# kdavila/lecturemath

Measured on AMD Instinct MI355X. Metric: frames/sec end-to-end binarize+CC+group @1080p, higher is better.
Workload: dtype u8

## Files before the change

### include/lecturemath_amd.h

```cpp
#ifndef LECTUREMATH_AMD_H
#define LECTUREMATH_AMD_H

#include <stdint.h>

#ifdef __cplusplus
extern "C" {
#endif

#define LM_OK 0
#define LM_ERR_ARG 1
#define LM_ERR_HIP 2
#define LM_ERR_CAPACITY 3
#define LM_ERR_STATE 4

typedef struct LmCtx LmCtx;
typedef struct LmStream LmStream;

int lm_abi_version(void);
const char* lm_last_error(void);
int lm_is_device_build(void);


int CC_AgeBoundaries(int* labels, float* ages, int width, int height, int count_labels,
                     int* out_mins_y, int* out_maxs_y, int* out_mins_x, int* out_maxs_x,
// ... 35 lines not shown
int lm_stream_push_records(LmStream* s, const uint8_t* d_binary, int n_frames, int32_t* d_labels, void* stream);
int lm_stream_match(LmStream* s, int n_frames, void* stream);
int lm_stream_push_labelled(LmStream* s, int n_frames, void* stream);

int lm_stream_run_logits(LmStream* s, const float* d_logits, int n_frames, int batch, uint8_t* d_binary, int32_t* d_labels, int thr,
                         int do_match, int schedule, void* stream_wide, void* stream_match);

int lm_stream_pack_size(LmStream* s, int first_frame, int n_frames, int64_t* h_bytes, void* stream);
int lm_stream_pack(LmStream* s, int first_frame, int n_frames, void* d_buf, int64_t bytes, void* stream);
int lm_stream_append_packed(LmStream* s, const void* d_buf, int64_t bytes, void* stream);

int lm_stream_assign_bytes(LmStream* s, int64_t* bytes, void* stream);
int lm_stream_export_assign(LmStream* s, void* d_out, int64_t bytes, void* stream);
int lm_stream_import_assign(LmStream* s, const void* d_in, int64_t bytes, void* stream);

int lm_stream_match_stats(LmStream* s, int64_t* out5, void* stream);

int lm_stream_counters(LmStream* s, int64_t* h_out7, void* stream);

int lm_stream_import(LmStream* s, const int32_t* h_rec, const int64_t* h_frame_off, const int64_t* h_crop_off,
                     const uint32_t* h_crop, int n_frames, int64_t n_cc, int64_t n_crop_words, int n_unique,
                     int64_t tempo_count, const int32_t* h_active, const int32_t* h_active_cc, const int32_t* h_active_last,
                     int n_active, int n_matched, void* stream);

int lm_stream_read(LmStream* s, int32_t* h_rec, int64_t* h_frame_off, int64_t* h_crop_off, uint32_t* h_crop,
                   int32_t* h_active, void* stream);

typedef struct LmGroups LmGroups;

LmGroups* lm_group_run(LmStream* s, int max_gap, int min_times, int t_window, double min_recall, double img_threshold,
                       int reconstruct_tables, void* stream);
// ... 63 lines not shown
```

### lecturemath_amd/csrc/lm_api.hip

```cpp
#include "lm_common.h"
#include "lm_stream.h"

#include <stdarg.h>
#include <stdlib.h>
#include <stdio.h>
#include <string.h>

#include "../../include/lecturemath_amd.h"

#include "lm_cc_kernels.hip"
#include "lm_match_kernels.hip"
#include "lm_match_batch.hip"
#include "lm_group.hip"
#include "lm_fcn.hip"
#include "lm_fcn2.hip"

static thread_local char g_err[512] = "";

void lm_set_error(const char* fmt, ...)
{
    va_list ap;
    va_start(ap, fmt);
    vsnprintf(g_err, sizeof(g_err), fmt, ap);
    va_end(ap);
// ... 479 lines not shown
    if (!ok) lm_set_error("CC_AgeBoundaries: device copy/launch failed");
    (void)hipFree(d_out);
    return 0;
}

extern "C" void lm_stream_destroy(LmStream* s)
{
    if (!s) return;
    void* ptrs[] = {s->cc, s->assign, s->frame_cc_off, s->crop, s->chash, s->active_cc, s->active_box, s->active_last, s->active, s->counters, s->best,
                    s->batch_cc_base, s->batch_word_base};
    for (void* p : ptrs)
        if (p) (void)hipFree(p);
    if (s->mb) {
        LmMatchBatch* m = s->mb;
        void* mp[] = {m->nt_cnt, m->nt_src, m->tlast, m->tcur[0], m->tcur[1], m->ftile_all, m->nt_foff, m->nt_list, m->cls, m->troot, m->rootpos, m->ftile, m->s_prefix, m->tcount[0], m->tcount[1], m->toff[0], m->toff[1], m->pairs[0], m->pairs[1], m->pair_u[0],
                      m->pair_u[1], m->sidx, m->s_list, m->s_box, m->newpos, m->n_src, m->ttab, m->tkey, m->twin, m->big[0], m->big[1], m->n_big};
        for (void* p : mp)
            if (p) (void)hipFree(p);
        delete m;
    }
    for (int i = 0; i < s->n_run_events; i++) (void)hipEventDestroy(s->run_events[i]);
    free(s->run_events);
    if (s->rd_scratch) (void)hipFree(s->rd_scratch);
    if (s->garena) (void)hipFree(s->garena);
    if (s->gpin) (void)hipHostFree(s->gpin);
    delete s;
}

extern "C" int lm_stream_set_min_pixels(LmStream* s, int min_pixels)
{
    if (!s || min_pixels < 0) { lm_set_error("lm_stream_set_min_pixels: bad arguments"); return LM_ERR_ARG; }
    s->min_pixels = min_pixels;
    return LM_OK;
}

extern "C" int lm_stream_reset(LmStream* s, void* stream)
{
    if (!s) { lm_set_error("lm_stream_reset: null stream"); return LM_ERR_ARG; }
    LM_HIP(hipMemsetAsync(s->counters, 0, sizeof(LmCounters), (hipStream_t)stream));
    LM_HIP(hipMemsetAsync(s->best, 0xff, (size_t)s->ctx->g.cap * sizeof(unsigned long long), (hipStream_t)stream));
    LM_HIP(hipMemsetAsync(s->frame_cc_off, 0, sizeof(long long), (hipStream_t)stream));
    LM_HIP(hipMemsetAsync(s->chash, 0, (size_t)s->cap_cc * sizeof(uint32_t), (hipStream_t)stream));
    if (s->mb) LM_HIP(hipMemsetAsync(s->mb->ttab, 0xff, (size_t)LM_MB_TTAB * sizeof(unsigned long long), (hipStream_t)stream));
    s->frames_pushed = 0;
    s->frames_matched = 0;
    s->tempo_B = 0;
    return LM_OK;
}

extern "C" LmStream* lm_stream_create(LmCtx* ctx, int max_frames, int64_t max_ccs, int64_t max_crop_words, int max_uniques,
                                      double min_recall, double min_precision, int max_gap, int min_pixels)
{
    if (!ctx || max_frames <= 0 || max_ccs <= 0 || max_crop_words <= 0 || max_uniques <= 0) {
        lm_set_error("lm_stream_create: bad arguments");
        return nullptr;
    }
    LmStream* s = new LmStream();
    memset(s, 0, sizeof(*s));
// ... 47 lines not shown
            rc |= lm_alloc(&m->pairs[k], (size_t)m->cap_pairs);
            rc |= lm_alloc(&m->pair_u[k], (size_t)m->cap_pairs);
        }
        rc |= lm_alloc(&m->sidx, (size_t)max_ccs);
        rc |= lm_alloc(&m->s_list, (size_t)max_ccs);
        rc |= lm_alloc(&m->s_box, (size_t)max_ccs);
        rc |= lm_alloc(&m->newpos, (size_t)max_ccs);
        rc |= lm_alloc(&m->n_src, (size_t)1);
        rc |= lm_alloc(&m->ttab, (size_t)LM_MB_TTAB);
        rc |= lm_alloc(&m->tkey, (size_t)max_ccs);
        rc |= lm_alloc(&m->twin, (size_t)max_ccs);
        m->cap_big = 1u << 16;
        rc |= lm_alloc(&m->big[0], (size_t)m->cap_big);
        rc |= lm_alloc(&m->big[1], (size_t)m->cap_big);
        rc |= lm_alloc(&m->n_big, (size_t)2);
#if !LM_HIP_EMULATED
        if (rc == LM_OK &&
            hipFuncSetAttribute((const void*)lm_k_mb_resolve, hipFuncAttributeMaxDynamicSharedMemorySize, (int)LM_MB_RESOLVE_SMEM) != hipSuccess)
            rc = LM_ERR_HIP;
#endif
        const char* e = getenv("LM_MATCH_PER_FRAME");
        s->match_per_frame = (e && atoi(e) == 1) ? 1 : 0;
    }
    if (rc == LM_OK && hipMemset(s->mb->twin, 0, (size_t)max_ccs) != hipSuccess) rc = LM_ERR_HIP;
    if (rc == LM_OK) rc = lm_stream_reset(s, nullptr);
    if (rc == LM_OK && hipStreamSynchronize(nullptr) != hipSuccess) rc = LM_ERR_HIP;
    if (rc != LM_OK) {
        lm_stream_destroy(s);
        return nullptr;
    }
// ... 28 lines not shown
    const dim3 gj(LM_HIP_EMULATED ? 2 : 128, LM_HIP_EMULATED ? 2 : LM_MB_JY), gt(LM_HIP_EMULATED ? 2 : 1024), ge(LM_HIP_EMULATED ? 2 : 2048), gb(LM_HIP_EMULATED ? 2 : 1024);
    for (int done = 0; done < n;) {
        const int B = (n - done < LM_MB_MAX_FRAMES) ? n - done : LM_MB_MAX_FRAMES;
        const int f = f0 + done;
        s->last_match_frames = B;
        const int twins = (s->min_recall <= 1.0 && s->min_precision <= 1.0) ? 1 : 0;
        if (twins) {
            const dim3 gc(LM_HIP_EMULATED ? 2 : 256);
            hipLaunchKernelGGL(lm_k_mb_twin_insert, gc, dim3(256), 0, st, s->cc, s->chash, s->frame_cc_off, f, B, s->counters, mb);
            hipLaunchKernelGGL(lm_k_mb_twin_probe, gc, dim3(256), 0, st, s->cc, s->frame_cc_off, f, B, s->counters, mb, s->max_gap);
            hipLaunchKernelGGL(lm_k_mb_twin_cmp, ge, dim3(256), 0, st, s->cc, s->crop, s->frame_cc_off, f, B, s->counters, mb);
            hipLaunchKernelGGL(lm_k_mb_twin_final, gc, dim3(256), 0, st, s->cc, s->frame_cc_off, f, B, s->counters, mb);
        }
        hipLaunchKernelGGL(lm_k_mb_nt, dim3(B + 1), dim3(1024), 0, st, s->frame_cc_off, f, B, s->active, s->active_cc, s->active_box, s->active_last,
                           s->counters, mb, s->max_gap, twins);
        hipLaunchKernelGGL((lm_k_mb_join<0, 0>), gj, dim3(256), 0, st, s->cc, s->frame_cc_off, f, B, s->active_box, s->active_cc, s->counters, mb);
        hipLaunchKernelGGL((lm_k_mb_join<0, 1>), gj, dim3(256), 0, st, s->cc, s->frame_cc_off, f, B, s->active_box, s->active_cc, s->counters, mb);
        hipLaunchKernelGGL((lm_k_mb_eval<0>), ge, dim3(256), 0, st, s->cc, s->crop, s->frame_cc_off, f, B, s->active_last, s->counters, mb,
                           s->min_recall, s->min_precision, s->max_gap);
        hipLaunchKernelGGL((lm_k_mb_eval_big<0>), gb, dim3(256), 0, st, s->cc, s->crop, s->active_last, s->counters, mb, s->min_recall, s->min_precision,
                           s->max_gap);
        hipLaunchKernelGGL(lm_k_mb_sources, dim3(1), dim3(1024), 0, st, s->cc, s->frame_cc_off, f, B, s->counters, mb);
        hipLaunchKernelGGL((lm_k_mb_join<1, 0>), gj, dim3(256), 0, st, s->cc, s->frame_cc_off, f, B, s->active_box, s->active_cc, s->counters, mb);
        hipLaunchKernelGGL((lm_k_mb_join<1, 1>), gj, dim3(256), 0, st, s->cc, s->frame_cc_off, f, B, s->active_box, s->active_cc, s->counters, mb);
        hipLaunchKernelGGL((lm_k_mb_eval<1>), ge, dim3(256), 0, st, s->cc, s->crop, s->frame_cc_off, f, B, s->active_last, s->counters, mb,
                           s->min_recall, s->min_precision, s->max_gap);
        hipLaunchKernelGGL((lm_k_mb_eval_big<1>), gb, dim3(256), 0, st, s->cc, s->crop, s->active_last, s->counters, mb, s->min_recall, s->min_precision,
                           s->max_gap);
        if (ev_pre && done + B >= n) (void)hipEventRecord(ev_pre, st);
        hipLaunchKernelGGL(lm_k_mb_resolve, dim3(1), dim3(LM_MB_RT), LM_MB_RESOLVE_SMEM, st, s->cc, s->frame_cc_off, f, B, s->active, s->active_cc,
                           s->active_box, s->active_last, s->counters, s->assign, mb, s->max_gap, s->cap_uniq);
        if (defer_tempo && done + B >= n) { s->tempo_f0 = f; s->tempo_B = B; }
        else
            hipLaunchKernelGGL(lm_k_mb_tempo, gt, dim3(256), 0, st, s->cc, s->frame_cc_off, f, B, s->active_box, s->active_cc, s->active_last,
                               s->counters, mb, s->max_gap, s->active, s->assign);
        done += B;
    }
}

// ... 142 lines not shown
    return LM_OK;
}

extern "C" int lm_stream_match(LmStream* s, int n_frames, void* stream)
{
    if (!s || n_frames < 0 || s->frames_matched + n_frames > s->frames_pushed) {
        lm_set_error("lm_stream_match: %d frames requested, %d pushed, %d matched", n_frames, s ? s->frames_pushed : 0, s ? s->frames_matched : 0);
        return LM_ERR_ARG;
    }
    lm_launch_match_frames(s, s->frames_matched, n_frames, (hipStream_t)stream);
    s->frames_matched += n_frames;
    LM_HIP(hipGetLastError());
    return LM_OK;
}

extern "C" int lm_stream_match_stats(LmStream* s, int64_t* out5, void* stream)
{
    if (!s || !out5 || !s->mb) { lm_set_error("lm_stream_match_stats: bad arguments"); return LM_ERR_ARG; }
    hipStream_t st = (hipStream_t)stream;
    const LmMatchBatch* m = s->mb;
    const int B = s->last_match_frames;
    int32_t nsrc = 0, nt = 0;
    uint32_t ta = 0, tb = 0;
    if (B > 0) {
        LM_HIP(hipMemcpyAsync(&nsrc, m->n_src, 4, hipMemcpyDeviceToHost, st));
        LM_HIP(hipMemcpyAsync(&nt, m->ftile + B, 4, hipMemcpyDeviceToHost, st));
        LM_HIP(hipStreamSynchronize(st));
        if (nt > 0) {
            LM_HIP(hipMemcpyAsync(&ta, m->toff[0] + nt, 4, hipMemcpyDeviceToHost, st));
            LM_HIP(hipMemcpyAsync(&tb, m->toff[1] + nt, 4, hipMemcpyDeviceToHost, st));
            LM_HIP(hipStreamSynchronize(st));
        }
    }
    out5[0] = nsrc; out5[1] = nt; out5[2] = ta; out5[3] = tb; out5[4] = B;
    return LM_OK;
}

__global__ void __launch_bounds__(1024) lm_k_compact_active(int32_t* __restrict__ active, int32_t* __restrict__ active_cc,
                                                            unsigned long long* __restrict__ active_box, int32_t* __restrict__ active_last,
                                                            LmCounters* __restrict__ cnt, int max_gap)
{
    if (cnt->error) return;
    const int f = cnt->n_matched;
    const int nA = cnt->n_active;
    if (f <= 1) return;
    unsigned kept = 0;
    for (int base = 0; base < nA; base += 1024) {
        int i = base + (int)threadIdx.x;
        int32_t u = 0, uc = 0, ul = 0;
// ... 371 lines not shown
```

### lecturemath_amd/csrc/lm_match_batch.hip

```cpp
#include "lm_stream.h"

#define LM_MB_TILE 64
#define LM_MB_JY 8
#define LM_MB_TTAB (1 << 18)
#ifndef LM_MB_CHUNK
#define LM_MB_CHUNK 1024
#endif
#define LM_MB_MAX_FRAMES 64
#define LM_MB_BIGPAIR 2048
#ifndef LM_MB_CH
#define LM_MB_CH 2048
#endif
#define LM_MB_LA 16384
#define LM_MB_LS 16384
#ifndef LM_MB_PFA
#define LM_MB_PFA 2
#endif
#ifndef LM_MB_PFB
#define LM_MB_PFB 1
#endif
#define LM_MB_RESOLVE_SMEM ((size_t)LM_MB_CH * 8 + (size_t)LM_MB_LA * 4 + (size_t)LM_MB_LS * 4)

struct LmMatchBatch {
    int32_t* ftile;
    int32_t* ftile_all;
    int32_t* nt_foff;
    int32_t* nt_list;
    int32_t* cls;
    int32_t* troot;
    int32_t* rootpos;
    int32_t* nt_cnt;
    int32_t* nt_src;
    int32_t* tlast;
    int32_t* s_prefix;
    uint32_t* tcount[2];
    uint32_t* toff[2];
    uint32_t* tcur[2];
    uint2* pairs[2];
    int32_t* pair_u[2];
    int32_t* sidx;
    int32_t* s_list;
    unsigned long long* s_box;
    int32_t* newpos;
    int32_t* n_src;
    unsigned long long* ttab;
    uint32_t* tkey;
    uint8_t* twin;
    uint32_t* big[2];
    unsigned* n_big;
    uint32_t cap_big;
    uint32_t cap_pairs;
    int cap_tiles;
};

LM_DEV bool lm_mb_alive(int f, int last, int max_gap) { return f <= 1 || (f - 1) - last < max_gap; }

typedef short lm_s16x2 __attribute__((ext_vector_type(2)));
struct alignas(16) lm_u64x2 { unsigned long long x, y; };
LM_DEV unsigned long long lm_box_as_cc(unsigned long long b)
{
    const unsigned x0 = (unsigned)(b & 0xffff), x1 = (unsigned)((b >> 16) & 0xffff), y0 = (unsigned)((b >> 32) & 0xffff), y1 = (unsigned)(b >> 48);
    return (unsigned long long)(x0 | ((0u - x1) << 16)) | ((unsigned long long)(y0 | ((0u - y1) << 16)) << 32);
}
LM_DEV unsigned long long lm_box_as_src(unsigned long long b)
// ... 106 lines not shown
        if (wid == 0) {
            const unsigned v = s_tab[lane];
            const unsigned incl = lm_wave_incl_scan(v);
            s_tab[lane] = incl - v;
            if (lane == 63) s_tot = incl;
        }
        __syncthreads();
#pragma unroll
        for (int k = 0; k < LM_MB_NT_R; k++) {
            const int flag = (int)((fm >> k) & 1u);
            const unsigned long long bal = __ballot(flag);
            const long long i = base + (long long)k * 1024 + threadIdx.x;
            if (flag) {
                const unsigned o = carry + s_tab[k * 16 + wid] + (unsigned)__popcll(bal & lm_lowmask_excl(lane));
                mb.nt_list[o] = (int32_t)i; mb.cls[i] = (int32_t)o; mb.tlast[o] = -1; mb.sidx[i] = -2;
            }
        }
        carry += s_tot;
        __syncthreads();
    }
}

LM_DEV int lm_mb_tile_frame(const int32_t* __restrict__ ftile, int B, int t)
{
    const int lane = lm_lane();
    const unsigned long long le = __ballot(lane < B && ftile[lane] <= t);
    return 63 - __clzll((long long)le);
}

template <int SRC, int FILL>
__global__ void __launch_bounds__(256) lm_k_mb_join(const LmCcRec* __restrict__ cc, const long long* __restrict__ frame_cc_off, int f0,
                                                    int B, const unsigned long long* __restrict__ active_box,
                                                    const int32_t* __restrict__ active_cc, LmCounters* __restrict__ cnt, LmMatchBatch mb)
{
    __shared__ __attribute__((aligned(16))) unsigned long long s_sbox[LM_MB_CHUNK + 4];
    __shared__ int s_spos[LM_MB_CHUNK];
    __shared__ int s_ub[4];
    __shared__ int s_nsurv;
    __shared__ unsigned s_count, s_base;
    if (cnt->error) return;
    const int nt = mb.ftile[B];
    const unsigned long long* src_box = SRC == 0 ? active_box : mb.s_box;
    const int32_t* src_cc = SRC == 0 ? active_cc : mb.s_list;
    const int ccl = (int)(threadIdx.x & 63), q = (int)(threadIdx.x >> 6);
    for (int t = blockIdx.x; t < nt; t += gridDim.x) {
        const int b = lm_mb_tile_frame(mb.ftile, B, t);
        const int n_all = SRC == 0 ? cnt->n_active : mb.s_prefix[b];
        const int s_lo = (int)((long long)n_all * blockIdx.y / gridDim.y), s_hi = (int)((long long)n_all * (blockIdx.y + 1) / gridDim.y);
        const int k_first = mb.nt_foff[b] + (t - mb.ftile[b]) * LM_MB_TILE;
        const int ncc = (mb.nt_foff[b + 1] - k_first < LM_MB_TILE) ? mb.nt_foff[b + 1] - k_first : LM_MB_TILE;
        __syncthreads();
        if (threadIdx.x == 0) { s_ub[0] = 0x7fff; s_ub[1] = -1; s_ub[2] = 0x7fff; s_ub[3] = -1; s_count = 0; }
        unsigned off = 0;
        if (FILL) {
            unsigned part = 0;
            for (int i = threadIdx.x; i < t; i += 256) part += mb.tcount[SRC][i];
// ... 78 lines not shown
                    } else {
                        mycount += hit ? 1u : 0u;
                    }
                }
            }
            if (!FILL) {
                if (mycount) atomicAdd(&s_count, mycount);
                __syncthreads();
                if (threadIdx.x == 0) {
                    if (s_count) atomicAdd(&mb.tcount[SRC][t], s_count);
                    mb.tcur[SRC][(size_t)t * LM_MB_JY + blockIdx.y] = s_count;
                }
                __syncthreads();
            }
        }
    }
}

template <int SRC>
__global__ void __launch_bounds__(256) lm_k_mb_eval(const LmCcRec* __restrict__ cc, const uint32_t* __restrict__ crop,
                                                    const long long* __restrict__ frame_cc_off, int f0, int B,
                                                    const int32_t* __restrict__ active_last, LmCounters* __restrict__ cnt,
                                                    LmMatchBatch mb, double min_recall, double min_precision, int max_gap)
{
    if (cnt->error) return;
    const int nt = mb.ftile[B];
    const unsigned total = nt > 0 ? mb.toff[SRC][nt] : 0u;
    const long long C0 = frame_cc_off[f0];
    if (SRC == 0) {
        const long long C1 = frame_cc_off[f0 + B];
// ... 30 lines not shown
        if (big && sub == 0) slot = atomicAdd(&mb.n_big[SRC], 1u);
        slot = (unsigned)__shfl((int)slot, 0, 8);
        const bool deferred = big && slot < mb.cap_big;
        if (deferred && sub == 0) mb.big[SRC][slot] = p;
        if (live && possible && !deferred) {
            for (int y = is.y0 + sub; y <= is.y1; y += 8) {
                const unsigned long long ra = rec.crop_off + (unsigned long long)((y - rec.min_y) * is.anw + (is.wc0 - is.awx0));
                const unsigned long long ru = urec.crop_off + (unsigned long long)((y - urec.min_y) * is.unw + (is.wc0 - is.uwx0));
                for (int j = 0; j < is.nwc; j++) m += __popc(crop[ra + j] & crop[ru + j]);
            }
        }
#pragma unroll
        for (int d = 4; d >= 1; d >>= 1) m += __shfl_xor(m, d, 8);
        if (live && possible && !deferred && sub == 0 && lm_accept(m, rec.size, urec.size, min_recall, min_precision)) {
            mb.pairs[SRC][p].x = pr.x | 0x80000000u;
            if (SRC == 0 && lm_mb_alive(rec.frame, active_last[pr.y], max_gap)) mb.sidx[ci] = -1;
        }
    }
}

template <int SRC>
__global__ void __launch_bounds__(256) lm_k_mb_eval_big(const LmCcRec* __restrict__ cc, const uint32_t* __restrict__ crop,
                                                        const int32_t* __restrict__ active_last, LmCounters* __restrict__ cnt, LmMatchBatch mb,
                                                        double min_recall, double min_precision, int max_gap)
{
    __shared__ int s_sum;
    if (cnt->error) return;
    const unsigned n = mb.n_big[SRC] < mb.cap_big ? mb.n_big[SRC] : mb.cap_big;
    for (unsigned b = blockIdx.x; b < n; b += gridDim.x) {
        const unsigned p = mb.big[SRC][b];
        const uint2 pr = mb.pairs[SRC][p];
        const long long ci = (long long)mb.nt_list[pr.x];
        const LmCcRec rec = cc[ci], urec = cc[mb.pair_u[SRC][p]];
        const LmIsect is = lm_isect(rec, urec);
        if (threadIdx.x == 0) s_sum = 0;
        __syncthreads();
        int m = lm_overlap_words(rec, urec, is, crop, (int)threadIdx.x, 256);
        m = lm_wave_sum(m);
        if (lm_lane() == 0 && m) atomicAdd(&s_sum, m);
        __syncthreads();
        if (threadIdx.x == 0 && lm_accept(s_sum, rec.size, urec.size, min_recall, min_precision)) {
            mb.pairs[SRC][p].x = pr.x | 0x80000000u;
            if (SRC == 0 && lm_mb_alive(rec.frame, active_last[pr.y], max_gap)) mb.sidx[ci] = -1;
        }
        __syncthreads();
    }
}

__global__ void __launch_bounds__(256) lm_k_mb_twin_insert(const LmCcRec* __restrict__ cc, const uint32_t* __restrict__ chash,
                                                           const long long* __restrict__ frame_cc_off, int f0, int B,
                                                           LmCounters* __restrict__ cnt, LmMatchBatch mb)
{
    if (cnt->error) return;
    const long long C0 = frame_cc_off[f0], C1 = frame_cc_off[f0 + B];
    const long long n = C1 - C0;
    if (blockIdx.x == 0 && threadIdx.x < LM_MB_MAX_FRAMES) mb.nt_cnt[threadIdx.x] = 0;
    if (n * 2 > LM_MB_TTAB) return;
    for (long long i = (long long)blockIdx.x * blockDim.x + threadIdx.x; i < n; i += (long long)gridDim.x * blockDim.x) {
// ... 189 lines not shown
            k = lm_cc_of_word(cc, c0, n, w, k0);
            contrib = lm_mix32(crop[w] + 0x9e3779b9u * (unsigned)(w - cc[c0 + k].crop_off));
        }
        const bool same = live && k == k0;
        const unsigned wsum = lm_wave_sum(same ? contrib : 0u);
        if (lane == 0 && live) atomicAdd(&chash[c0 + k0], wsum);
        if (live && !same) atomicAdd(&chash[c0 + k], contrib);
    }
}

#define LM_MB_SRC_R 8

__global__ void __launch_bounds__(1024) lm_k_mb_sources(const LmCcRec* __restrict__ cc, const long long* __restrict__ frame_cc_off,
                                                        int f0, int B, LmCounters* __restrict__ cnt, LmMatchBatch mb)
{
    __shared__ unsigned s_tab[LM_MB_SRC_R * 16];
    __shared__ unsigned s_tot;
    if (cnt->error) return;
    const int nNT = mb.nt_foff[B];
    const int lane = lm_lane(), wid = (int)(threadIdx.x >> 6);
    unsigned carry = 0;
    for (int base = 0; base < nNT; base += 1024 * LM_MB_SRC_R) {
        int ci[LM_MB_SRC_R], v[LM_MB_SRC_R];
#pragma unroll
        for (int k = 0; k < LM_MB_SRC_R; k++) {
            const int e = base + k * 1024 + (int)threadIdx.x;
            ci[k] = (e < nNT) ? mb.nt_list[e] : -1;
        }
#pragma unroll
        for (int k = 0; k < LM_MB_SRC_R; k++) v[k] = (ci[k] >= 0) ? mb.sidx[ci[k]] : 0;
        unsigned fm = 0;
#pragma unroll
        for (int k = 0; k < LM_MB_SRC_R; k++) {
            const int flag = v[k] == -2;
            fm |= (unsigned)flag << k;
            const unsigned long long bal = __ballot(flag);
            if (lane == 0) s_tab[k * 16 + wid] = (unsigned)__popcll(bal);
        }
        __syncthreads();
        if (wid == 0) {
            constexpr int PER = LM_MB_SRC_R * 16 / 64;
            unsigned loc[PER], sum = 0;
#pragma unroll
            for (int j = 0; j < PER; j++) { loc[j] = s_tab[lane * PER + j]; sum += loc[j]; }
            const unsigned incl = lm_wave_incl_scan(sum);
            unsigned run = incl - sum;
#pragma unroll
            for (int j = 0; j < PER; j++) { s_tab[lane * PER + j] = run; run += loc[j]; }
            if (lane == 63) s_tot = incl;
        }
        __syncthreads();
#pragma unroll
        for (int k = 0; k < LM_MB_SRC_R; k++) {
            const int flag = (int)((fm >> k) & 1u);
            const unsigned long long bal = __ballot(flag);
            const int e = base + k * 1024 + (int)threadIdx.x;
            if (e < nNT) {
                const unsigned o = carry + s_tab[k * 16 + wid] + (unsigned)__popcll(bal & lm_lowmask_excl(lane));
                mb.rootpos[e] = (int32_t)o;
                mb.nt_src[e] = flag ? (int32_t)o : -1;
                if (flag) {
                    mb.sidx[ci[k]] = (int32_t)o;
                    mb.s_list[o] = ci[k];
                    mb.s_box[o] = lm_pack_box(cc[ci[k]]);
                    mb.newpos[o] = -1;
                }
            }
        }
        carry += s_tot;
        __syncthreads();
    }
    if (threadIdx.x == 0) *mb.n_src = (int)carry;
    if ((int)threadIdx.x <= B) {
        const int e = mb.nt_foff[threadIdx.x];
        mb.s_prefix[threadIdx.x] = (e < nNT) ? mb.rootpos[e] : (int)carry;
    }
}

#ifndef LM_MB_RT
#define LM_MB_RT 1024
#endif
#define LM_MB_ITEMS (LM_MB_CH / LM_MB_RT)
#define LM_MB_SCAN_DIRECT 512

LM_DEV void lm_mb_prefetch(const LmMatchBatch& mb, unsigned pA0, unsigned pA1, unsigned pB0, unsigned pB1, int n0, int n,
                           uint2 (&ra)[LM_MB_PFA], uint2 (&rb)[LM_MB_PFB], int (&rs)[LM_MB_ITEMS], int (&rc)[LM_MB_ITEMS], int (&rt)[LM_MB_ITEMS])
{
#pragma unroll
    for (int k = 0; k < LM_MB_PFA; k++) {
        const unsigned pa = pA0 + (unsigned)k * (unsigned)LM_MB_RT + threadIdx.x;
// ... 24 lines not shown
    if (lm_mb_alive(f, last, max_gap)) atomicMin(&s_best[idx], pr.y);
}

LM_DEV void lm_mb_pair_new(uint2 pr, int f, int max_gap, unsigned rel0, unsigned nch, unsigned* s_best, const int* s_last, const int* s_newpos,
                           const int32_t* __restrict__ active_last, const int32_t* __restrict__ newpos)
{
    if (!(pr.x >> 31)) return;
    const unsigned idx = (pr.x & 0x7fffffffu) - rel0;
    if (idx >= nch) return;
    const int pos = pr.y < LM_MB_LS ? s_newpos[pr.y] : newpos[pr.y];
    if (pos < 0) return;
    const int last = pos < LM_MB_LA ? s_last[pos] : active_last[pos];
    if (lm_mb_alive(f, last, max_gap)) atomicMin(&s_best[idx], (unsigned)pos);
}

__global__ void __launch_bounds__(LM_MB_RT) lm_k_mb_resolve(const LmCcRec* __restrict__ cc, const long long* __restrict__ frame_cc_off,
                                                            int f0, int B, int32_t* __restrict__ active, int32_t* __restrict__ active_cc,
                                                            unsigned long long* __restrict__ active_box, int32_t* __restrict__ active_last,
                                                            LmCounters* __restrict__ cnt, int32_t* __restrict__ assign, LmMatchBatch mb,
                                                            int max_gap, int cap_uniq)
{
    LM_DYN_SMEM(smem);
    unsigned* s_best2 = (unsigned*)smem;
    int* s_last = (int*)(smem + (size_t)LM_MB_CH * 8);
    int* s_newpos = s_last + LM_MB_LA;
    __shared__ int s_n0[LM_MB_MAX_FRAMES + 1];
    __shared__ unsigned s_tA[LM_MB_MAX_FRAMES + 1], s_tB[LM_MB_MAX_FRAMES + 1];
    __shared__ int s_fail;
    __shared__ unsigned s_wsum[LM_MB_RT / 64];
    if (cnt->error) return;
    const int nt = mb.ftile[B];
    const int nA0 = cnt->n_active;
    const int nS = *mb.n_src;
    int nA = nA0;
    int nU = cnt->n_uniq;
    const bool lds_only = (long long)nA0 + nS <= LM_MB_LA && nS <= LM_MB_LS;
    if (threadIdx.x == 0) s_fail = 0;
    if ((int)threadIdx.x <= B) {
        s_n0[threadIdx.x] = mb.nt_foff[threadIdx.x];
        const int t = mb.ftile[threadIdx.x];
        s_tA[threadIdx.x] = nt > 0 ? mb.toff[0][t] : 0u;
        s_tB[threadIdx.x] = nt > 0 ? mb.toff[1][t] : 0u;
    }
    for (int i = threadIdx.x; i < nA0 && i < LM_MB_LA; i += LM_MB_RT) s_last[i] = active_last[i];
    for (int k = threadIdx.x; k < nS && k < LM_MB_LS; k += LM_MB_RT) s_newpos[k] = -1;
    for (int i = threadIdx.x; i < 2 * LM_MB_CH; i += LM_MB_RT) s_best2[i] = 0xffffffffu;
    int bb = 0;
    __syncthreads();
    uint2 ra[LM_MB_PFA], rb[LM_MB_PFB];
    int rs[LM_MB_ITEMS], rc[LM_MB_ITEMS], rt[LM_MB_ITEMS];
    lm_mb_prefetch(mb, s_tA[0], s_tA[1], s_tB[0], s_tB[1], s_n0[0], s_n0[1] - s_n0[0], ra, rb, rs, rc, rt);

    for (int b = 0; b < B; b++) {
        const int f = f0 + b;
        const int n0 = s_n0[b], n = s_n0[b + 1] - n0;
        if (n == 0) {
            if (b + 1 < B) lm_mb_prefetch(mb, s_tA[b + 1], s_tA[b + 2], s_tB[b + 1], s_tB[b + 2], s_n0[b + 1], s_n0[b + 2] - s_n0[b + 1], ra, rb, rs, rc, rt);
            continue;
        }
        const bool single = n <= LM_MB_CH;
        const unsigned pA0 = s_tA[b], pA1 = s_tA[b + 1], pB0 = s_tB[b], pB1 = s_tB[b + 1];
        for (int cb = 0; cb < n; cb += LM_MB_CH) {
            const int nch = (n - cb < LM_MB_CH) ? n - cb : LM_MB_CH;
            const unsigned rel0 = (unsigned)(n0 + cb);
            unsigned* s_best = s_best2 + bb * LM_MB_CH;
            if (single) {
#pragma unroll
                for (int k = 0; k < LM_MB_PFA; k++)
                    if (ra[k].y != 0xffffffffu) lm_mb_pair_old(ra[k], f, max_gap, rel0, (unsigned)nch, s_best, s_last, active_last);
#pragma unroll
                for (int k = 0; k < LM_MB_PFB; k++)
                    if (rb[k].y != 0xffffffffu) lm_mb_pair_new(rb[k], f, max_gap, rel0, (unsigned)nch, s_best, s_last, s_newpos, active_last, mb.newpos);
            }
            for (unsigned p = pA0 + (single ? (unsigned)LM_MB_PFA * (unsigned)LM_MB_RT : 0u) + threadIdx.x; p < pA1; p += LM_MB_RT)
                lm_mb_pair_old(mb.pairs[0][p], f, max_gap, rel0, (unsigned)nch, s_best, s_last, active_last);
            for (unsigned p = pB0 + (single ? (unsigned)LM_MB_PFB * (unsigned)LM_MB_RT : 0u) + threadIdx.x; p < pB1; p += LM_MB_RT)
                lm_mb_pair_new(mb.pairs[1][p], f, max_gap, rel0, (unsigned)nch, s_best, s_last, s_newpos, active_last, mb.newpos);
            int cur_s[LM_MB_ITEMS], cur_c[LM_MB_ITEMS], cur_t[LM_MB_ITEMS];
#pragma unroll
            for (int k = 0; k < LM_MB_ITEMS; k++) {
                const int i = (int)threadIdx.x * LM_MB_ITEMS + k;
                const bool on = i < nch;
                cur_s[k] = single ? rs[k] : (on ? mb.nt_src[n0 + cb + i] : -1);
                cur_c[k] = single ? rc[k] : (on ? mb.nt_list[n0 + cb + i] : 0);
                cur_t[k] = single ? rt[k] : (on ? mb.tlast[n0 + cb + i] : -1);
            }
            if (cb + LM_MB_CH >= n && b + 1 < B)
                lm_mb_prefetch(mb, s_tA[b + 1], s_tA[b + 2], s_tB[b + 1], s_tB[b + 2], s_n0[b + 1], s_n0[b + 2] - s_n0[b + 1], ra, rb, rs, rc, rt);
            if (lds_only) lm_lds_barrier(); else __syncthreads();
            for (int i = threadIdx.x; i < LM_MB_CH; i += LM_MB_RT) s_best2[(bb ^ 1) * LM_MB_CH + i] = 0xffffffffu;
            unsigned isnew[LM_MB_ITEMS], mine = 0;
#pragma unroll
            for (int k = 0; k < LM_MB_ITEMS; k++) {
                const int i = (int)threadIdx.x * LM_MB_ITEMS + k;
                isnew[k] = 0;
                if (i < nch) {
                    const unsigned best = s_best[i];
                    if (best != 0xffffffffu) {
                        const int upto = cur_t[k] > f ? cur_t[k] : f;
                        assign[cur_c[k]] = -2 - (int32_t)best;
                        if (best < LM_MB_LA) atomicMax(&s_last[best], upto);
                        atomicMax(&active_last[best], upto);
                    } else {
// ... 37 lines not shown
                    active_last[pos] = upto;
                    if (pos < LM_MB_LA) s_last[pos] = upto;
                    mb.newpos[src] = pos;
                    if (src < LM_MB_LS) s_newpos[src] = pos;
                } else {
                    s_fail = idx < cap_uniq ? LM_ERR_STATE : LM_ERR_CAPACITY;
                }
                o++;
            }
            nA += (int)tot;
            nU += (int)tot;
            bb ^= 1;
            if (lds_only) lm_lds_barrier(); else __syncthreads();
        }
    }
    __syncthreads();
    if (!s_fail) {
        for (int pos = nA0 + (int)threadIdx.x; pos < nA; pos += LM_MB_RT) active_box[pos] = lm_pack_box(cc[active_cc[pos]]);
    }
    __syncthreads();
    if (threadIdx.x == 0) {
        if (s_fail) {
            cnt->error = s_fail;
        } else {
            cnt->n_uniq = nU;
            cnt->n_active = nA;
            cnt->n_matched = f0 + B;
        }
    }
}

#ifndef LM_MB_TCHUNK
#define LM_MB_TCHUNK 4096
#endif
#define LM_MB_TUN 8

__global__ void __launch_bounds__(256) lm_k_mb_tempo(const LmCcRec* __restrict__ cc, const long long* __restrict__ frame_cc_off, int f0, int B,
                                                     const unsigned long long* __restrict__ active_box, const int32_t* __restrict__ active_cc,
                                                     const int32_t* __restrict__ active_last, LmCounters* __restrict__ cnt, LmMatchBatch mb,
                                                     int max_gap, const int32_t* __restrict__ active, int32_t* __restrict__ assign)
{
    __shared__ __attribute__((aligned(16))) unsigned long long s_sbox[LM_MB_TCHUNK + 4];
// ... 100 lines not shown
```

Before: 74340.

## Pre-resolve unambiguous batch matches early and add single-wave resolve path

The accept step now records, for each new CC, the minimum accepted active candidate overall and the minimum among alive candidates. When these agree, the CC's assignment is committed in the second join pass, so the sequential resolve kernel only sees a compacted list of the remaining CCs. Frames with few remaining CCs and pairs are handled by one wavefront that uses ballots instead of block-wide barriers, and frames with nothing left are skipped. It also adds per-frame match statistics written by the device and exported through an expanded match_stats API. The cost is extra atomics, several new buffers and a serial stats pass at the end of resolve.

```diff
diff --git a/include/lecturemath_amd.h b/include/lecturemath_amd.h
--- a/include/lecturemath_amd.h
+++ b/include/lecturemath_amd.h
@@ -73,7 +73,8 @@
 int lm_stream_export_assign(LmStream* s, void* d_out, int64_t bytes, void* stream);
 int lm_stream_import_assign(LmStream* s, const void* d_in, int64_t bytes, void* stream);
 
-int lm_stream_match_stats(LmStream* s, int64_t* out5, void* stream);
+#define LM_MATCH_STATS_LEN 272
+int lm_stream_match_stats(LmStream* s, int64_t* out, void* stream);
 
 int lm_stream_counters(LmStream* s, int64_t* h_out7, void* stream);
 
diff --git a/lecturemath_amd/csrc/lm_api.hip b/lecturemath_amd/csrc/lm_api.hip
--- a/lecturemath_amd/csrc/lm_api.hip
+++ b/lecturemath_amd/csrc/lm_api.hip
@@ -517,7 +517,8 @@
     if (s->mb) {
         LmMatchBatch* m = s->mb;
         void* mp[] = {m->nt_cnt, m->nt_src, m->tlast, m->tcur[0], m->tcur[1], m->ftile_all, m->nt_foff, m->nt_list, m->cls, m->troot, m->rootpos, m->ftile, m->s_prefix, m->tcount[0], m->tcount[1], m->toff[0], m->toff[1], m->pairs[0], m->pairs[1], m->pair_u[0],
-                      m->pair_u[1], m->sidx, m->s_list, m->s_box, m->newpos, m->n_src, m->ttab, m->tkey, m->twin, m->big[0], m->big[1], m->n_big};
+                      m->pair_u[1], m->sidx, m->s_list, m->s_box, m->newpos, m->n_src, m->ttab, m->tkey, m->twin, m->big[0], m->big[1], m->n_big,
+                      m->amin, m->amin_alive, m->has_b, m->rpos, m->r_ent, m->r_foff, m->stats};
         for (void* p : mp)
             if (p) (void)hipFree(p);
         delete m;
@@ -545,6 +546,7 @@
     LM_HIP(hipMemsetAsync(s->frame_cc_off, 0, sizeof(long long), (hipStream_t)stream));
     LM_HIP(hipMemsetAsync(s->chash, 0, (size_t)s->cap_cc * sizeof(uint32_t), (hipStream_t)stream));
     if (s->mb) LM_HIP(hipMemsetAsync(s->mb->ttab, 0xff, (size_t)LM_MB_TTAB * sizeof(unsigned long long), (hipStream_t)stream));
+    if (s->mb) LM_HIP(hipMemsetAsync(s->mb->stats, 0, sizeof(LmMatchStats), (hipStream_t)stream));
     s->frames_pushed = 0;
     s->frames_matched = 0;
     s->tempo_B = 0;
@@ -622,6 +624,13 @@
         rc |= lm_alloc(&m->big[0], (size_t)m->cap_big);
         rc |= lm_alloc(&m->big[1], (size_t)m->cap_big);
         rc |= lm_alloc(&m->n_big, (size_t)2);
+        rc |= lm_alloc(&m->amin, (size_t)max_ccs);
+        rc |= lm_alloc(&m->amin_alive, (size_t)max_ccs);
+        rc |= lm_alloc(&m->has_b, (size_t)max_ccs);
+        rc |= lm_alloc(&m->rpos, (size_t)max_ccs);
+        rc |= lm_alloc(&m->r_ent, (size_t)max_ccs);
+        rc |= lm_alloc(&m->r_foff, (size_t)max_frames + 2);
+        rc |= lm_alloc(&m->stats, (size_t)1);
 #if !LM_HIP_EMULATED
         if (rc == LM_OK &&
             hipFuncSetAttribute((const void*)lm_k_mb_resolve, hipFuncAttributeMaxDynamicSharedMemorySize, (int)LM_MB_RESOLVE_SMEM) != hipSuccess)
@@ -680,15 +689,19 @@
         }
         hipLaunchKernelGGL(lm_k_mb_nt, dim3(B + 1), dim3(1024), 0, st, s->frame_cc_off, f, B, s->active, s->active_cc, s->active_box, s->active_last,
                            s->counters, mb, s->max_gap, twins);
-        hipLaunchKernelGGL((lm_k_mb_join<0, 0>), gj, dim3(256), 0, st, s->cc, s->frame_cc_off, f, B, s->active_box, s->active_cc, s->counters, mb);
-        hipLaunchKernelGGL((lm_k_mb_join<0, 1>), gj, dim3(256), 0, st, s->cc, s->frame_cc_off, f, B, s->active_box, s->active_cc, s->counters, mb);
+        hipLaunchKernelGGL((lm_k_mb_join<0, 0>), gj, dim3(256), 0, st, s->cc, s->frame_cc_off, f, B, s->active_box, s->active_cc, s->counters, mb,
+                           s->active_last, s->assign);
+        hipLaunchKernelGGL((lm_k_mb_join<0, 1>), gj, dim3(256), 0, st, s->cc, s->frame_cc_off, f, B, s->active_box, s->active_cc, s->counters, mb,
+                           s->active_last, s->assign);
         hipLaunchKernelGGL((lm_k_mb_eval<0>), ge, dim3(256), 0, st, s->cc, s->crop, s->frame_cc_off, f, B, s->active_last, s->counters, mb,
                            s->min_recall, s->min_precision, s->max_gap);
         hipLaunchKernelGGL((lm_k_mb_eval_big<0>), gb, dim3(256), 0, st, s->cc, s->crop, s->active_last, s->counters, mb, s->min_recall, s->min_precision,
                            s->max_gap);
         hipLaunchKernelGGL(lm_k_mb_sources, dim3(1), dim3(1024), 0, st, s->cc, s->frame_cc_off, f, B, s->counters, mb);
-        hipLaunchKernelGGL((lm_k_mb_join<1, 0>), gj, dim3(256), 0, st, s->cc, s->frame_cc_off, f, B, s->active_box, s->active_cc, s->counters, mb);
-        hipLaunchKernelGGL((lm_k_mb_join<1, 1>), gj, dim3(256), 0, st, s->cc, s->frame_cc_off, f, B, s->active_box, s->active_cc, s->counters, mb);
+        hipLaunchKernelGGL((lm_k_mb_join<1, 0>), gj, dim3(256), 0, st, s->cc, s->frame_cc_off, f, B, s->active_box, s->active_cc, s->counters, mb,
+                           s->active_last, s->assign);
+        hipLaunchKernelGGL((lm_k_mb_join<1, 1>), gj, dim3(256), 0, st, s->cc, s->frame_cc_off, f, B, s->active_box, s->active_cc, s->counters, mb,
+                           s->active_last, s->assign);
         hipLaunchKernelGGL((lm_k_mb_eval<1>), ge, dim3(256), 0, st, s->cc, s->crop, s->frame_cc_off, f, B, s->active_last, s->counters, mb,
                            s->min_recall, s->min_precision, s->max_gap);
         hipLaunchKernelGGL((lm_k_mb_eval_big<1>), gb, dim3(256), 0, st, s->cc, s->crop, s->active_last, s->counters, mb, s->min_recall, s->min_precision,
@@ -861,9 +874,9 @@
     return LM_OK;
 }
 
-extern "C" int lm_stream_match_stats(LmStream* s, int64_t* out5, void* stream)
-{
-    if (!s || !out5 || !s->mb) { lm_set_error("lm_stream_match_stats: bad arguments"); return LM_ERR_ARG; }
+extern "C" int lm_stream_match_stats(LmStream* s, int64_t* out, void* stream)
+{
+    if (!s || !out || !s->mb) { lm_set_error("lm_stream_match_stats: bad arguments"); return LM_ERR_ARG; }
     hipStream_t st = (hipStream_t)stream;
     const LmMatchBatch* m = s->mb;
     const int B = s->last_match_frames;
@@ -879,7 +892,14 @@
             LM_HIP(hipStreamSynchronize(st));
         }
     }
-    out5[0] = nsrc; out5[1] = nt; out5[2] = ta; out5[3] = tb; out5[4] = B;
+    out[0] = nsrc; out[1] = nt; out[2] = ta; out[3] = tb; out[4] = B;
+    LmMatchStats h;
+    LM_HIP(hipMemcpyAsync(&h, m->stats, sizeof(h), hipMemcpyDeviceToHost, st));
+    LM_HIP(hipStreamSynchronize(st));
+    for (int i = 0; i < 5; i++) { out[5 + i] = h.last[i]; out[10 + i] = h.sum[i]; }
+    out[15] = h.batches;
+    for (int b = 0; b < LM_MB_MAX_FRAMES; b++)
+        for (int i = 0; i < 4; i++) out[16 + 4 * b + i] = b < B ? h.fr[b][i] : 0;
     return LM_OK;
 }
 
diff --git a/lecturemath_amd/csrc/lm_match_batch.hip b/lecturemath_amd/csrc/lm_match_batch.hip
--- a/lecturemath_amd/csrc/lm_match_batch.hip
+++ b/lecturemath_amd/csrc/lm_match_batch.hip
@@ -21,6 +21,24 @@
 #endif
 #define LM_MB_RESOLVE_SMEM ((size_t)LM_MB_CH * 8 + (size_t)LM_MB_LA * 4 + (size_t)LM_MB_LS * 4)
 
+#define LM_MB_NONE 0xffffffffu
+#define LM_MB_WPAIRS 1024
+
+struct alignas(16) LmResEnt {
+    int32_t cc;
+    int32_t src;
+    int32_t tlast;
+    int32_t k;
+};
+
+struct LmMatchStats {
+    long long sum[5];
+    long long batches;
+    int32_t last[5];
+    int32_t pad;
+    int32_t fr[LM_MB_MAX_FRAMES][4];
+};
+
 struct LmMatchBatch {
     int32_t* ftile;
     int32_t* ftile_all;
@@ -29,6 +47,7 @@
     int32_t* cls;
     int32_t* troot;
     int32_t* rootpos;
+    int32_t* rpos;
     int32_t* nt_cnt;
     int32_t* nt_src;
     int32_t* tlast;
@@ -48,6 +67,12 @@
     uint8_t* twin;
     uint32_t* big[2];
     unsigned* n_big;
+    uint32_t* amin;
+    uint32_t* amin_alive;
+    int32_t* has_b;
+    LmResEnt* r_ent;
+    int32_t* r_foff;
+    LmMatchStats* stats;
     uint32_t cap_big;
     uint32_t cap_pairs;
     int cap_tiles;
@@ -184,6 +209,7 @@
             if (flag) {
                 const unsigned o = carry + s_tab[k * 16 + wid] + (unsigned)__popcll(bal & lm_lowmask_excl(lane));
                 mb.nt_list[o] = (int32_t)i; mb.cls[i] = (int32_t)o; mb.tlast[o] = -1; mb.sidx[i] = -2;
+                mb.amin[o] = LM_MB_NONE; mb.amin_alive[o] = LM_MB_NONE; mb.has_b[o] = 0;
             }
         }
         carry += s_tot;
@@ -201,7 +227,8 @@
 template <int SRC, int FILL>
 __global__ void __launch_bounds__(256) lm_k_mb_join(const LmCcRec* __restrict__ cc, const long long* __restrict__ frame_cc_off, int f0,
                                                     int B, const unsigned long long* __restrict__ active_box,
-                                                    const int32_t* __restrict__ active_cc, LmCounters* __restrict__ cnt, LmMatchBatch mb)
+                                                    const int32_t* __restrict__ active_cc, LmCounters* __restrict__ cnt, LmMatchBatch mb,
+                                                    int32_t* __restrict__ active_last, int32_t* __restrict__ assign)
 {
     __shared__ __attribute__((aligned(16))) unsigned long long s_sbox[LM_MB_CHUNK + 4];
     __shared__ int s_spos[LM_MB_CHUNK];
@@ -210,6 +237,17 @@
     __shared__ unsigned s_count, s_base;
     if (cnt->error) return;
     const int nt = mb.ftile[B];
+    if (SRC == 1 && !FILL) {
+        const int nNT = mb.nt_foff[B];
+        for (int k = (int)((blockIdx.y * gridDim.x + blockIdx.x) * 256u + threadIdx.x); k < nNT; k += (int)(gridDim.x * gridDim.y * 256u)) {
+            const unsigned a = mb.amin[k];
+            if (a == LM_MB_NONE || a != mb.amin_alive[k]) continue;
+            const long long ci = (long long)mb.nt_list[k];
+            const int f = cc[ci].frame, tl = mb.tlast[k];
+            assign[ci] = -2 - (int32_t)a;
+            atomicMax(&active_last[a], tl > f ? tl : f);
+        }
+    }
     const unsigned long long* src_box = SRC == 0 ? active_box : mb.s_box;
     const int32_t* src_cc = SRC == 0 ? active_cc : mb.s_list;
     const int ccl = (int)(threadIdx.x & 63), q = (int)(threadIdx.x >> 6);
@@ -318,6 +356,17 @@
                 __syncthreads();
             }
         }
+    }
+}
+
+template <int SRC>
+LM_DEV void lm_mb_accepted(const LmMatchBatch& mb, uint2 pr, long long ci, int frame, const int32_t* __restrict__ active_last, int max_gap)
+{
+    if (SRC == 0) {
+        atomicMin(&mb.amin[pr.x], pr.y);
+        if (lm_mb_alive(frame, active_last[pr.y], max_gap)) { atomicMin(&mb.amin_alive[pr.x], pr.y); mb.sidx[ci] = -1; }
+    } else {
+        mb.has_b[pr.x] = 1;
     }
 }
 
@@ -378,7 +427,7 @@
         for (int d = 4; d >= 1; d >>= 1) m += __shfl_xor(m, d, 8);
         if (live && possible && !deferred && sub == 0 && lm_accept(m, rec.size, urec.size, min_recall, min_precision)) {
             mb.pairs[SRC][p].x = pr.x | 0x80000000u;
-            if (SRC == 0 && lm_mb_alive(rec.frame, active_last[pr.y], max_gap)) mb.sidx[ci] = -1;
+            lm_mb_accepted<SRC>(mb, pr, ci, rec.frame, active_last, max_gap);
         }
     }
 }
@@ -405,7 +454,7 @@
         __syncthreads();
         if (threadIdx.x == 0 && lm_accept(s_sum, rec.size, urec.size, min_recall, min_precision)) {
             mb.pairs[SRC][p].x = pr.x | 0x80000000u;
-            if (SRC == 0 && lm_mb_alive(rec.frame, active_last[pr.y], max_gap)) mb.sidx[ci] = -1;
+            lm_mb_accepted<SRC>(mb, pr, ci, rec.frame, active_last, max_gap);
         }
         __syncthreads();
     }
@@ -625,40 +674,50 @@
 __global__ void __launch_bounds__(1024) lm_k_mb_sources(const LmCcRec* __restrict__ cc, const long long* __restrict__ frame_cc_off,
                                                         int f0, int B, LmCounters* __restrict__ cnt, LmMatchBatch mb)
 {
-    __shared__ unsigned s_tab[LM_MB_SRC_R * 16];
-    __shared__ unsigned s_tot;
+    __shared__ unsigned s_tab[2 * LM_MB_SRC_R * 16];
+    __shared__ unsigned s_tot, s_rtot;
     if (cnt->error) return;
     const int nNT = mb.nt_foff[B];
     const int lane = lm_lane(), wid = (int)(threadIdx.x >> 6);
-    unsigned carry = 0;
+    unsigned carry = 0, rcarry = 0;
     for (int base = 0; base < nNT; base += 1024 * LM_MB_SRC_R) {
         int ci[LM_MB_SRC_R], v[LM_MB_SRC_R];
+        unsigned am[LM_MB_SRC_R], aa[LM_MB_SRC_R];
+        int so[LM_MB_SRC_R];
 #pragma unroll
         for (int k = 0; k < LM_MB_SRC_R; k++) {
             const int e = base + k * 1024 + (int)threadIdx.x;
             ci[k] = (e < nNT) ? mb.nt_list[e] : -1;
         }
 #pragma unroll
-        for (int k = 0; k < LM_MB_SRC_R; k++) v[k] = (ci[k] >= 0) ? mb.sidx[ci[k]] : 0;
-        unsigned fm = 0;
+        for (int k = 0; k < LM_MB_SRC_R; k++) {
+            const int e = base + k * 1024 + (int)threadIdx.x;
+            v[k] = (ci[k] >= 0) ? mb.sidx[ci[k]] : 0;
+            am[k] = (ci[k] >= 0) ? mb.amin[e] : 0u;
+            aa[k] = (ci[k] >= 0) ? mb.amin_alive[e] : 0u;
+        }
+        unsigned fm = 0, rm = 0;
 #pragma unroll
         for (int k = 0; k < LM_MB_SRC_R; k++) {
             const int flag = v[k] == -2;
+            const int res = ci[k] >= 0 && (am[k] == LM_MB_NONE || am[k] != aa[k]);
             fm |= (unsigned)flag << k;
-            const unsigned long long bal = __ballot(flag);
-            if (lane == 0) s_tab[k * 16 + wid] = (unsigned)__popcll(bal);
-        }
-        __syncthreads();
-        if (wid == 0) {
+            rm |= (unsigned)res << k;
+            const unsigned long long bal = __ballot(flag), rbal = __ballot(res);
+            if (lane == 0) { s_tab[k * 16 + wid] = (unsigned)__popcll(bal); s_tab[(LM_MB_SRC_R + k) * 16 + wid] = (unsigned)__popcll(rbal); }
+        }
+        __syncthreads();
+        if (wid < 2) {
             constexpr int PER = LM_MB_SRC_R * 16 / 64;
+            unsigned* tab = s_tab + wid * LM_MB_SRC_R * 16;
             unsigned loc[PER], sum = 0;
 #pragma unroll
-            for (int j = 0; j < PER; j++) { loc[j] = s_tab[lane * PER + j]; sum += loc[j]; }
+            for (int j = 0; j < PER; j++) { loc[j] = tab[lane * PER + j]; sum += loc[j]; }
             const unsigned incl = lm_wave_incl_scan(sum);
             unsigned run = incl - sum;
 #pragma unroll
-            for (int j = 0; j < PER; j++) { s_tab[lane * PER + j] = run; run += loc[j]; }
-            if (lane == 63) s_tot = incl;
+            for (int j = 0; j < PER; j++) { tab[lane * PER + j] = run; run += loc[j]; }
+            if (lane == 63) { if (wid == 0) s_tot = incl; else s_rtot = incl; }
         }
         __syncthreads();
 #pragma unroll
@@ -670,6 +729,7 @@
                 const unsigned o = carry + s_tab[k * 16 + wid] + (unsigned)__popcll(bal & lm_lowmask_excl(lane));
                 mb.rootpos[e] = (int32_t)o;
                 mb.nt_src[e] = flag ? (int32_t)o : -1;
+                so[k] = flag ? (int)o : -1;
                 if (flag) {
                     mb.sidx[ci[k]] = (int32_t)o;
                     mb.s_list[o] = ci[k];
@@ -678,13 +738,30 @@
                 }
             }
         }
+#pragma unroll
+        for (int k = 0; k < LM_MB_SRC_R; k++) {
+            const int res = (int)((rm >> k) & 1u);
+            const unsigned long long rbal = __ballot(res);
+            const int e = base + k * 1024 + (int)threadIdx.x;
+            if (e < nNT) {
+                const unsigned ro = rcarry + s_tab[(LM_MB_SRC_R + k) * 16 + wid] + (unsigned)__popcll(rbal & lm_lowmask_excl(lane));
+                mb.rpos[e] = (int32_t)ro;
+                if (res) {
+                    LmResEnt r;
+                    r.cc = ci[k]; r.src = so[k]; r.tlast = mb.tlast[e]; r.k = e;
+                    mb.r_ent[ro] = r;
+                }
+            }
+        }
         carry += s_tot;
+        rcarry += s_rtot;
         __syncthreads();
     }
     if (threadIdx.x == 0) *mb.n_src = (int)carry;
     if ((int)threadIdx.x <= B) {
         const int e = mb.nt_foff[threadIdx.x];
         mb.s_prefix[threadIdx.x] = (e < nNT) ? mb.rootpos[e] : (int)carry;
+        mb.r_foff[threadIdx.x] = (e < nNT) ? mb.rpos[e] : (int)rcarry;
     }
 }
 
@@ -739,6 +816,71 @@
     if (lm_mb_alive(f, last, max_gap)) atomicMin(&s_best[idx], (unsigned)pos);
 }
 
+LM_DEV void lm_mb_wave_frame(const LmMatchBatch& mb, int f, int max_gap, int cap_uniq, int r0, int r, unsigned pA0, unsigned pA1, unsigned pB0,
+                             unsigned pB1, int* s_last, int* s_newpos, int* s_fail, int32_t* __restrict__ active, int32_t* __restrict__ active_cc,
+                             int32_t* __restrict__ active_last, int32_t* __restrict__ assign, int& nA, int& nU)
+{
+    const int lane = lm_lane();
+    const bool have = lane < r;
+    LmResEnt e;
+    e.cc = 0; e.src = -1; e.tlast = -1; e.k = -1;
+    if (have) e = mb.r_ent[r0 + lane];
+    unsigned best = LM_MB_NONE;
+#pragma unroll
+    for (int src = 0; src < 2; src++) {
+        const unsigned p0 = src ? pB0 : pA0, p1 = src ? pB1 : pA1;
+        for (unsigned base = p0; base < p1; base += 256) {
+            uint2 q[4];
+#pragma unroll
+            for (int u = 0; u < 4; u++) {
+                const unsigned p = base + (unsigned)u * 64u + (unsigned)lane;
+                q[u] = (p < p1) ? mb.pairs[src][p] : make_uint2(0u, 0u);
+            }
+#pragma unroll
+            for (int u = 0; u < 4; u++) {
+                bool ok = (q[u].x >> 31) != 0;
+                int pos = (int)q[u].y;
+                if (ok && src) { pos = s_newpos[q[u].y]; ok = pos >= 0; }
+                if (ok) ok = lm_mb_alive(f, s_last[pos], max_gap);
+                unsigned long long todo = __ballot(ok);
+                while (todo) {
+                    const int l = __ffsll((long long)todo) - 1;
+                    const int kk = __shfl((int)(q[u].x & 0x7fffffffu), l), pp = __shfl(pos, l);
+                    if (kk == e.k && (unsigned)pp < best) best = (unsigned)pp;
+                    todo &= todo - 1;
+                }
+            }
+        }
+    }
+    const int upto = e.tlast > f ? e.tlast : f;
+    const bool isnew = have && best == LM_MB_NONE;
+    if (have && !isnew) {
+        assign[e.cc] = -2 - (int32_t)best;
+        atomicMax(&s_last[best], upto);
+        atomicMax(&active_last[best], upto);
+    }
+    const unsigned long long nb = __ballot(isnew);
+    const int o = (int)__popcll(nb & lm_lowmask_excl(lane)), tot = (int)__popcll(nb);
+    if (isnew) {
+        const long long idx = (long long)nU + o;
+        if (idx < cap_uniq && e.src >= 0) {
+            const int pos = nA + o;
+            assign[e.cc] = (int32_t)idx;
+            active[pos] = (int32_t)idx;
+            active_cc[pos] = e.cc;
+            active_last[pos] = upto;
+            if (pos < LM_MB_LA) s_last[pos] = upto;
+            mb.newpos[e.src] = pos;
+            if (e.src < LM_MB_LS) s_newpos[e.src] = pos;
+        } else {
+            *s_fail = idx < cap_uniq ? LM_ERR_STATE : LM_ERR_CAPACITY;
+        }
+    }
+    nA += tot;
+    nU += tot;
+    LM_WAVE_SYNC();
+}
+
 __global__ void __launch_bounds__(LM_MB_RT) lm_k_mb_resolve(const LmCcRec* __restrict__ cc, const long long* __restrict__ frame_cc_off,
                                                             int f0, int B, int32_t* __restrict__ active, int32_t* __restrict__ active_cc,
                                                             unsigned long long* __restrict__ active_box, int32_t* __restrict__ active_last,
@@ -751,7 +893,9 @@
     int* s_newpos = s_last + LM_MB_LA;
     __shared__ int s_n0[LM_MB_MAX_FRAMES + 1];
     __shared__ unsigned s_tA[LM_MB_MAX_FRAMES + 1], s_tB[LM_MB_MAX_FRAMES + 1];
-    __shared__ int s_fail;
+    __shared__ int s_r0[LM_MB_MAX_FRAMES + 1];
+    __shared__ int s_cn[LM_MB_MAX_FRAMES], s_path[LM_MB_MAX_FRAMES];
+    __shared__ int s_fail, s_nAU[2];
     __shared__ unsigned s_wsum[LM_MB_RT / 64];
     if (cnt->error) return;
     const int nt = mb.ftile[B];
@@ -761,8 +905,10 @@
     int nU = cnt->n_uniq;
     const bool lds_only = (long long)nA0 + nS <= LM_MB_LA && nS <= LM_MB_LS;
     if (threadIdx.x == 0) s_fail = 0;
+    if ((int)threadIdx.x < LM_MB_MAX_FRAMES) s_cn[threadIdx.x] = 0;
     if ((int)threadIdx.x <= B) {
         s_n0[threadIdx.x] = mb.nt_foff[threadIdx.x];
+        s_r0[threadIdx.x] = mb.r_foff[threadIdx.x];
         const int t = mb.ftile[threadIdx.x];
         s_tA[threadIdx.x] = nt > 0 ? mb.toff[0][t] : 0u;
         s_tB[threadIdx.x] = nt > 0 ? mb.toff[1][t] : 0u;
@@ -772,17 +918,36 @@
     for (int i = threadIdx.x; i < 2 * LM_MB_CH; i += LM_MB_RT) s_best2[i] = 0xffffffffu;
     int bb = 0;
     __syncthreads();
+    if ((int)threadIdx.x < B) {
+        const int b = (int)threadIdx.x, r = s_r0[b + 1] - s_r0[b];
+        const unsigned np = (s_tA[b + 1] - s_tA[b]) + (s_tB[b + 1] - s_tB[b]);
+        s_path[b] = r == 0 ? 0 : (lds_only && r <= 64 && np <= LM_MB_WPAIRS) ? 1 : 2;
+    }
+    __syncthreads();
     uint2 ra[LM_MB_PFA], rb[LM_MB_PFB];
     int rs[LM_MB_ITEMS], rc[LM_MB_ITEMS], rt[LM_MB_ITEMS];
-    lm_mb_prefetch(mb, s_tA[0], s_tA[1], s_tB[0], s_tB[1], s_n0[0], s_n0[1] - s_n0[0], ra, rb, rs, rc, rt);
+    int pf = -1;
+    bool wave_ran = false;
 
     for (int b = 0; b < B; b++) {
         const int f = f0 + b;
+        const int path = s_path[b];
+        if (path == 0) continue;
+        if (path == 1) {
+            if (threadIdx.x < 64)
+                lm_mb_wave_frame(mb, f, max_gap, cap_uniq, s_r0[b], s_r0[b + 1] - s_r0[b], s_tA[b], s_tA[b + 1], s_tB[b], s_tB[b + 1], s_last, s_newpos,
+                                 &s_fail, active, active_cc, active_last, assign, nA, nU);
+            wave_ran = true;
+            continue;
+        }
+        if (wave_ran) {
+            if (threadIdx.x == 0) { s_nAU[0] = nA; s_nAU[1] = nU; }
+            lm_lds_barrier();
+            nA = s_nAU[0]; nU = s_nAU[1];
+            wave_ran = false;
+        }
         const int n0 = s_n0[b], n = s_n0[b + 1] - n0;
-        if (n == 0) {
-            if (b + 1 < B) lm_mb_prefetch(mb, s_tA[b + 1], s_tA[b + 2], s_tB[b + 1], s_tB[b + 2], s_n0[b + 1], s_n0[b + 2] - s_n0[b + 1], ra, rb, rs, rc, rt);
-            continue;
-        }
+        if (pf != b) lm_mb_prefetch(mb, s_tA[b], s_tA[b + 1], s_tB[b], s_tB[b + 1], n0, n, ra, rb, rs, rc, rt);
         const bool single = n <= LM_MB_CH;
         const unsigned pA0 = s_tA[b], pA1 = s_tA[b + 1], pB0 = s_tB[b], pB1 = s_tB[b + 1];
         for (int cb = 0; cb < n; cb += LM_MB_CH) {
@@ -810,8 +975,10 @@
                 cur_c[k] = single ? rc[k] : (on ? mb.nt_list[n0 + cb + i] : 0);
                 cur_t[k] = single ? rt[k] : (on ? mb.tlast[n0 + cb + i] : -1);
             }
-            if (cb + LM_MB_CH >= n && b + 1 < B)
+            if (cb + LM_MB_CH >= n && b + 1 < B && s_path[b + 1] == 2) {
                 lm_mb_prefetch(mb, s_tA[b + 1], s_tA[b + 2], s_tB[b + 1], s_tB[b + 2], s_n0[b + 1], s_n0[b + 2] - s_n0[b + 1], ra, rb, rs, rc, rt);
+                pf = b + 1;
+            }
             if (lds_only) lm_lds_barrier(); else __syncthreads();
             for (int i = threadIdx.x; i < LM_MB_CH; i += LM_MB_RT) s_best2[(bb ^ 1) * LM_MB_CH + i] = 0xffffffffu;
             unsigned isnew[LM_MB_ITEMS], mine = 0;
@@ -879,11 +1046,21 @@
             if (lds_only) lm_lds_barrier(); else __syncthreads();
         }
     }
+    if (wave_ran && threadIdx.x == 0) { s_nAU[0] = nA; s_nAU[1] = nU; }
     __syncthreads();
+    if (wave_ran) { nA = s_nAU[0]; nU = s_nAU[1]; }
     if (!s_fail) {
         for (int pos = nA0 + (int)threadIdx.x; pos < nA; pos += LM_MB_RT) active_box[pos] = lm_pack_box(cc[active_cc[pos]]);
+        for (int j = (int)threadIdx.x; j < s_r0[B]; j += LM_MB_RT) {
+            const LmResEnt e = mb.r_ent[j];
+            if (mb.amin[e.k] == LM_MB_NONE && !mb.has_b[e.k]) atomicAdd(&s_cn[cc[e.cc].frame - f0], 1);
+        }
     }
     __syncthreads();
+    if (!s_fail && (int)threadIdx.x < B) {
+        const int b = (int)threadIdx.x, n = s_n0[b + 1] - s_n0[b], r = s_r0[b + 1] - s_r0[b];
+        mb.stats->fr[b][0] = n; mb.stats->fr[b][1] = n - r; mb.stats->fr[b][2] = s_cn[b]; mb.stats->fr[b][3] = s_path[b];
+    }
     if (threadIdx.x == 0) {
         if (s_fail) {
             cnt->error = s_fail;
@@ -891,6 +1068,10 @@
             cnt->n_uniq = nU;
             cnt->n_active = nA;
             cnt->n_matched = f0 + B;
+            int v[5] = {s_n0[B], s_n0[B] - s_r0[B], 0, s_r0[B], 0};
+            for (int b = 0; b < B; b++) { v[2] += s_cn[b]; v[4] += s_path[b] == 2 ? 1 : 0; }
+            for (int i = 0; i < 5; i++) { mb.stats->last[i] = v[i]; mb.stats->sum[i] += v[i]; }
+            mb.stats->batches += 1;
         }
     }
 }
```

After: 74150. Within noise of the previous version (-0.3%).
